# mic-rud/Learned-Compression-of-Point-Cloud-Geometry-and-Attributes

Measured on AMD Instinct MI355X. Metric: encode+decode Mpoints/sec, higher is better.
Workload: dtype f32

## Files before the change

### include/pcc_hip.h

```cpp
#ifndef PCC_HIP_H
#define PCC_HIP_H

#include <stdint.h>

#ifdef __cplusplus
extern "C" {
#endif

#define PCC_OK 0
#define PCC_ERR_ARG (-1)
#define PCC_ERR_HIP (-2)
#define PCC_ERR_UNSUPPORTED (-3)
#define PCC_ERR_DATA (-4)

#define PCC_ACT_NONE 0
#define PCC_ACT_RELU 1
#define PCC_ACT_LEAKY_RELU 2

int pcc_version(void);
const char* pcc_last_error(void);
int pcc_device_count(void);
int pcc_device_name(int dev, char* out, int out_len);

int64_t pcc_hash_capacity(int64_t n);
// ... 17 lines not shown
int pcc_children(const int32_t* coords, int64_t n, int32_t ts, int32_t ksize, uint64_t* keys,
                 int32_t* vals, int64_t cap, int32_t* scratch, int32_t* out_coords,
                 int64_t* out_count, void* stream);

int pcc_augment_rotate(const int32_t* coords, int64_t n, const float* rot, int32_t nbatch, float half,
                       uint64_t* keys, int32_t* vals, int64_t cap, int32_t* scratch, int32_t* out_coords,
                       int32_t* out_src, int64_t* out_count, void* stream);

int32_t pcc_color_jitter_chunk(void);
int64_t pcc_color_jitter_scratch_bytes(int64_t n, int32_t nbatch);
int pcc_color_jitter(const float* rgb, int64_t n, const int64_t* offsets, int32_t nbatch, const float* params,
                     const int32_t* order, float* out, void* scratch, int64_t scratch_bytes, void* stream);

int pcc_voxelize(const float* xyz, const int32_t* batch, int64_t n, int32_t nbatch, const float* attr, int32_t c,
                 float origin_x, float origin_y, float origin_z, float voxel, int32_t rounding, uint64_t* keys,
                 int32_t* vals, int64_t cap, int32_t* scratch, int32_t* out_coords, int32_t* out_first,
                 int32_t* out_npts, int64_t* out_sum, int32_t* out_row, int64_t* out_count, void* stream);

int pcc_kernel_map(const int32_t* out_coords, int64_t n_out, const uint64_t* in_keys,
                   const int32_t* in_vals, int64_t in_cap, int32_t ksize, int32_t step,
                   int32_t sign, int32_t* nbr, uint32_t* row_mask, int64_t* pair_count,
                   void* stream);

int pcc_pair_count(const uint32_t* row_mask, int64_t n_out, int64_t* pair_count, void* stream);

int64_t pcc_order_scratch_bytes(int64_t n);
int pcc_order_rows_by_mask(const uint32_t* row_mask, const int32_t* coords, int64_t n,
                           int32_t block_log2, int32_t tensor_stride, int32_t* order, uint32_t* group_mask32,
                           void* scratch, int64_t scratch_bytes, void* stream);
int pcc_permute_map_rows(const int32_t* nbr, const int32_t* order, int64_t n, int32_t K, int32_t* nbr_sorted, void* stream);

int64_t pcc_small_map_max(void);
int32_t pcc_small_paths(int32_t mask);
int pcc_small_kernel_map(const int32_t* out_coords, int64_t n_out, const uint64_t* in_keys, const int32_t* in_vals, int64_t in_cap,
                         int32_t ksize, int32_t step, int32_t sign, int32_t* nbr, uint32_t* row_mask, int32_t* order,
                         uint32_t* group_mask32, void* scratch, int64_t scratch_bytes, void* stream);

int64_t pcc_conv_packed_elems(int32_t K, int32_t cin, int32_t cout);
int pcc_conv_pack_weights(const float* w, int32_t K, int32_t cin, int32_t cout, float* w_packed,
                          void* stream);
int pcc_conv_fwd(const float* fin, int64_t n_in, int32_t cin, const float* w, const float* w_packed,
                 const float* bias, const int32_t* nbr, const int32_t* order,
                 const uint32_t* group_mask32, int32_t K, float* fout, int64_t n_out, int32_t cout,
                 int32_t act, const float* film, const float* residual, void* stream);

int64_t pcc_conv_small_max(int64_t workgroups);

int pcc_conv_kernel_name(int32_t mode, int64_t n_in, int32_t cin, int32_t cout, int64_t n_out, int32_t K, int32_t has_nbr,
                         char* buf, int32_t len);

int64_t pcc_conv_packed_elems_bf16(int32_t K, int32_t cin, int32_t cout);
int pcc_conv_pack_weights_bf16(const float* w, int32_t K, int32_t cin, int32_t cout, uint16_t* w_packed, void* stream);
// ... 13 lines not shown
int64_t pcc_conv_packed_elems_x3(int32_t K, int32_t cin, int32_t cout);
int pcc_conv_pack_weights_x3(const float* w, int32_t K, int32_t cin, int32_t cout, uint16_t* w_packed, void* stream);
int pcc_conv_fwd_x3(const float* fin, int64_t n_in, int32_t cin, const uint16_t* w_packed, const float* bias,
                    const int32_t* nbr, const int32_t* order, const uint32_t* group_mask32, int32_t K, float* fout,
                    int64_t n_out, int32_t cout, int32_t act, const float* film, const float* residual, void* stream);

int pcc_im2col_thin(const float* fin, int32_t cin, const int32_t* nbr, int64_t n_out, int32_t K, float* out, int32_t k2,
                    void* stream);

int pcc_gather_sum_fwd(const float* scores, int32_t ld, const int32_t* nbr, int32_t K, int32_t cout,
                       const float* bias, float* out, int64_t n_out, int32_t act, void* stream);

int pcc_gather_rows(const float* src, int32_t c, const int32_t* idx, int64_t n, float* out,
                    int32_t accumulate, void* stream);

int pcc_scatter_rows(const float* src, int32_t c, const int32_t* idx, int64_t n, float* out,
                     void* stream);
int pcc_scatter_add_rows(const float* src, int32_t c, const int32_t* idx, int64_t n, float* out,
                         void* stream);

int pcc_compact_rows(const uint8_t* mask, int64_t n, const int32_t* coords, int32_t* out_coords,
                     const float* feats, int32_t c, float* out_feats, int32_t* new_index,
                     int32_t* scratch, int64_t* out_count, void* stream);

int64_t pcc_topk_state_elems(int32_t nbatch);
int pcc_topk_mask(const float* logits, int32_t ld, const int32_t* coords, int64_t n, int32_t nbatch,
                  const int32_t* k, uint8_t* mask, int32_t* state, void* stream);

int pcc_count_per_batch(const int32_t* coords, int64_t n, int32_t nbatch, int32_t* counts, void* stream);

int64_t pcc_sort_scratch_bytes(int64_t n);
int pcc_sort_coords(const int32_t* coords, int64_t n, int32_t* perm, void* scratch,
                    int64_t scratch_bytes, void* stream);

int pcc_kernel_map_transpose(const int32_t* nbr, int64_t n_out, int32_t K, int64_t n_in, int32_t* nbr_t,
                             uint32_t* row_mask_t, void* stream);
int64_t pcc_conv_wgrad_scratch_elems(int32_t K, int32_t cin, int32_t cout);
int pcc_conv_wgrad(const float* fin, int64_t n_in, int32_t cin, const float* dy, int64_t n_out, int32_t cout,
                   const int32_t* nbr, const int32_t* order, const uint32_t* group_mask32, int32_t K, float* dw,
                   float* scratch, int64_t scratch_elems, void* stream);
int pcc_conv_wgrad_kernel_name(int32_t bf16, int32_t K, int32_t cin, int32_t cout, int64_t n_out, char* buf, int32_t len,
                               int32_t* split, int32_t* partials);
int pcc_conv_wgrad_bf16(const uint16_t* fin, int64_t n_in, int32_t cin, const uint16_t* dy, int64_t n_out, int32_t cout,
                        const int32_t* nbr, const int32_t* order, const uint32_t* group_mask32, int32_t K, float* dw,
                        float* scratch, int64_t scratch_elems, void* stream);

// ... 116 lines not shown
```

### learned-compression-of-point-cloud-geometry-and-attributes_amd/blocks.py

```python
import os

import torch
import torch.nn as nn

from . import _threads
from . import sparse as sp
from .sparse import (ACT_NONE, ACT_RELU, ConvChain, CoordMap, MinkowskiConvolution,
                     MinkowskiGenerativeConvolutionTranspose, MinkowskiPruning, MinkowskiReLU, SparseTensor)


class _NonNegativeParametrizer(nn.Module):
    def __init__(self, minimum=0.0, reparam_offset=2 ** -18):
        super().__init__()
        pedestal = float(reparam_offset) ** 2
        self.register_buffer("pedestal", torch.tensor([pedestal]))
        self.lower_bound = _Bound((float(minimum) + pedestal) ** 0.5)


class _Bound(nn.Module):
    def __init__(self, bound):
        super().__init__()
        self.register_buffer("bound", torch.tensor([float(bound)]))


# ... 24 lines not shown

    def forward(self, x, condition):
        if condition.map is x.map:
            film = condition.F
        else:
            film = condition.features_at_coordinates(x.C)
        N = x.F.shape[1]
        if film.shape[1] == 2 and N != 1:
            film = torch.cat([film[:, :1].expand(-1, N), film[:, 1:].expand(-1, N)], dim=1).contiguous()
        h = self.conv_1(x, last_film=film if self.scale else None)
        return self.conv_2(h, last_residual=x.F)


def _start_prefetch(x_map, done_key, job, handoffs):
    if os.environ.get("PCC_PREFETCH_MAPS", "1") == "0" or torch.is_grad_enabled() or x_map._cache.get(done_key):
        return False
    dev = x_map.device
    main = torch.cuda.current_stream(dev)
    st = _threads.current()
    skey = (dev, main.cuda_stream)
    side = st.side_streams.get(skey)
    if side is None:
        side = st.side_streams[skey] = torch.cuda.Stream(device=dev)
    x_map.table()
    side.wait_stream(main)

    def run():
        try:
            with torch.cuda.stream(side):
                job(side)
        except BaseException as e:
            for h in handoffs:
                h.fail(e)
            raise

    if x_map.n >= PREFETCH_THREAD_MIN_ROWS:
        x_map._cache[("prefetch_job",)] = st.job_thread("pcc-map-prefetch", dev).submit(run)
    else:
        run()
    x_map._cache[done_key] = True
    return True


PREFETCH_THREAD_MIN_ROWS = 8192


def prefetch_up_maps(x_map):
    first = _threads.Handoff()

    def job(side):
        cand = x_map.up(3)
        x_map.mfma_kernel_map(cand, 3, True)
        first.set(side.record_event())
        cand.mfma_kernel_map(cand, 3)
        cand.kernel_map(cand, 3)
# ... 37 lines not shown
    last = level == -1 or level >= len(syncs)
    try:
        ev = (syncs[-1] if last else syncs[level - 1]).wait()
    except BaseException:
        x_map._cache.pop(("analysis_syncs",), None)
        x_map._cache.pop(("prefetch_job",), None)
        raise
    torch.cuda.current_stream(x_map.device).wait_event(ev)
    if last:
        x_map._cache.pop(("analysis_syncs",), None)
        _join_prefetch(x_map)


def _join_prefetch_first(x_map):
    first = x_map._cache.pop(("prefetch_first",), None)
    if first is None:
        return
    try:
        ev = first.wait()
    except BaseException:
        x_map._cache.pop(("prefetch_job",), None)
        raise
    torch.cuda.current_stream(x_map.device).wait_event(ev)


def _join_prefetch(x_map):
    x_map._cache.pop(("prefetch_first",), None)
    done = x_map._cache.pop(("prefetch_job",), None)
    if done is not None:
        done.wait()
    ev = x_map._cache.pop(("prefetch_event",), None)
    if ev is not None:
        torch.cuda.current_stream(x_map.device).wait_event(ev)


class GenerativeUpBlock(nn.Module):

    def __init__(self, N_in, N_out, predict=False, dense=True, condition_ablation=None):
        super().__init__()
        self.dense = dense
        self.condition_ablation = condition_ablation
        self.conv = MinkowskiGenerativeConvolutionTranspose(in_channels=N_in, out_channels=N_out, kernel_size=3,
                                                            stride=2, bias=True, dimension=3)
        self.conv_2 = ConvChain(_conv(N_out, N_out), MinkowskiReLU(), _conv(N_out, N_out))
        self.prune = MinkowskiPruning()
        self.predict = predict
        if predict:
            self.occ_predict = ConvChain(_conv(N_out, N_out), MinkowskiReLU(), _conv(N_out, N_out))

    def forward(self, x, coords=None, k=None, full_predictions=False):
        if not self.predict:
            return self._follow(x, coords)
        in_map = x.map
        _join_prefetch_first(in_map)
        x = self.conv(x)
        _join_prefetch(in_map)
        if self.dense and self.condition_ablation is None:
            x = self.conv_2(x)
        pred = self.occ_predict(x, last_out_channels=None if full_predictions else 1)
        nb = x.map._nbatch if x.map._nbatch is not None else x.map.nbatch
        mask = sp.topk_mask(pred.F, pred.C, k, nb)
        kept = min(max(int(k[0]), 0), x.map.n) if nb == 1 and len(k) == 1 and not torch.is_grad_enabled() else None
        coords_kept, feats_kept, _, _ = sp.compact_rows(mask, x.C, x.F, expected=kept)
        up_map = CoordMap(coords_kept, x.map.stride, nbatch=x.map._nbatch)
        x = SparseTensor(feats_kept, coordinate_map=up_map)
        if not self.dense and self.condition_ablation is None:
            x = self.conv_2(x)
        return x, pred, up_map

    def _follow(self, Q, up_map):
        if not isinstance(up_map, CoordMap):
            up_map = CoordMap(sp._as_int_coords(up_map), Q.map.stride // 2, nbatch=Q.map._nbatch)
        return self.conv(Q, out_map=up_map)


class ConditionEncoder(nn.Module):

    def __init__(self, C_in, N_scales, N_features, condition_ablation=None):
        super().__init__()
        self.num_stages = len(N_scales)
        self.condition_ablation = condition_ablation
        self.pre_conv = ConvChain(_conv(C_in, N_features[0]), MinkowskiReLU())
        self.conv_layers = nn.ModuleList()
        self.predict_layers = nn.ModuleList()
        self.down_layers = nn.ModuleList()
        for i in range(self.num_stages):
            down = _conv(N_features[i], N_features[i + 1], 3, 2)
# ... 34 lines not shown
```

### learned-compression-of-point-cloud-geometry-and-attributes_amd/csrc/coords.hip

```cpp
#include <stdarg.h>
#include <stdio.h>
#include <stdlib.h>

#include "common.h"
#include "first_rows.h"
#include "sort.h"

namespace pcc {

static thread_local char g_err[512] = "";
void set_error(const char* fmt, ...) {
    va_list ap;
    va_start(ap, fmt);
    vsnprintf(g_err, sizeof(g_err), fmt, ap);
    va_end(ap);
}
const char* last_error() { return g_err; }

constexpr int SCAN_BLOCK = 256;
constexpr int SCAN_ITEMS = 4;
constexpr int SCAN_TILE = SCAN_BLOCK * SCAN_ITEMS;

__device__ __forceinline__ int wave_inclusive_scan(int v, int lane) {
#pragma unroll
    for (int d = 1; d < 64; d <<= 1) {
        const int t = __shfl_up(v, d, 64);
        if (lane >= d) v += t;
    }
// ... 396 lines not shown
            kk[i] = keys[sl];
            vv[i] = vals[sl];
        }
        int idx = -1;
        bool open = true;
        const int lane_slots = (int)((mask + TABLE_PROBE_STEP) / TABLE_PROBE_STEP);
#pragma unroll
        for (int i = 0; i < 4; ++i) {
            if (!open) break;
            if (i + 1 >= lane_slots) break;
            if (kk[i] == key) { idx = vv[i]; open = false; }
            else if (kk[i] == KEY_EMPTY) { idx = -1; open = false; }
        }
        if (open) idx = table_find(keys, vals, mask, shift, key);
        nbr[row0 * 27 + e] = idx;
        if (idx >= 0) { atomicOr(&rm[lr], 1u << k); ++myhits; }
    }
    if (myhits) atomicAdd(&hits_s, myhits);
    __syncthreads();
    if (row_mask && threadIdx.x < nrows) row_mask[row0 + threadIdx.x] = rm[threadIdx.x];
    if (threadIdx.x == 0 && pair_count && !row_mask && hits_s) atomicAdd(pair_count, (unsigned long long)hits_s);
}

__global__ __launch_bounds__(256) void pair_count_kernel(const uint32_t* __restrict__ row_mask, int64_t n,
                                                         unsigned long long* __restrict__ pair_count) {
    __shared__ unsigned long long ws[4];
    unsigned long long v = 0;
    for (int64_t i = (int64_t)blockIdx.x * 256 + threadIdx.x; i < n; i += (int64_t)gridDim.x * 256) v += __popc(row_mask[i]);
#pragma unroll
    for (int d = 32; d >= 1; d >>= 1) v += __shfl_xor(v, d, 64);
    if ((threadIdx.x & 63) == 0) ws[threadIdx.x >> 6] = v;
    __syncthreads();
    if (threadIdx.x == 0) {
        const unsigned long long t = ws[0] + ws[1] + ws[2] + ws[3];
        if (t) atomicAdd(pair_count, t);
    }
}

__global__ __launch_bounds__(256) void gather_rows_kernel(const float* __restrict__ src, int c,
                                                          const int32_t* __restrict__ idx, int64_t n,
                                                          float* __restrict__ out, int accumulate) {
    const int64_t total = n * c;
    for (int64_t e = (int64_t)blockIdx.x * blockDim.x + threadIdx.x; e < total; e += (int64_t)gridDim.x * blockDim.x) {
        const int64_t r = e / c;
        const int col = (int)(e - r * c);
        const int32_t s = idx[r];
// ... 16 lines not shown

__global__ __launch_bounds__(256) void scatter_add_rows_kernel(const float* __restrict__ src, int c,
                                                               const int32_t* __restrict__ idx, int64_t n,
                                                               float* __restrict__ out) {
    const int64_t total = n * c;
    for (int64_t e = (int64_t)blockIdx.x * blockDim.x + threadIdx.x; e < total; e += (int64_t)gridDim.x * blockDim.x) {
        const int64_t r = e / c;
        const int col = (int)(e - r * c);
        const int32_t d = idx[r];
        if (d >= 0) atomicAdd(&out[(int64_t)d * c + col], src[e]);
    }
}

__global__ __launch_bounds__(256) void mask_to_flags(const uint8_t* __restrict__ mask, int64_t n,
                                                     int32_t* __restrict__ flags) {
    const int64_t i = (int64_t)blockIdx.x * blockDim.x + threadIdx.x;
    if (i < n) flags[i] = mask[i] ? 1 : 0;
}

__global__ __launch_bounds__(256) void compact_index_kernel(const uint8_t* __restrict__ mask,
                                                            const int32_t* __restrict__ pos, int64_t n,
                                                            const int32_t* __restrict__ coords,
                                                            int32_t* __restrict__ out_coords,
                                                            int32_t* __restrict__ new_index) {
    const int64_t i = (int64_t)blockIdx.x * blockDim.x + threadIdx.x;
    if (i >= n) return;
    const bool keep = mask[i] != 0;
    const int32_t p = pos[i];
    if (new_index) new_index[i] = keep ? p : -1;
    if (keep && coords) reinterpret_cast<int4*>(out_coords)[p] = reinterpret_cast<const int4*>(coords)[i];
}

__global__ __launch_bounds__(256) void compact_feats_kernel(const uint8_t* __restrict__ mask,
                                                            const int32_t* __restrict__ pos, int64_t n, int c,
                                                            const float* __restrict__ feats,
                                                            float* __restrict__ out_feats, int vec) {
    if (vec) {
        const int c4 = c >> 2;
        const int64_t total = n * c4;
        const float4* src = reinterpret_cast<const float4*>(feats);
        float4* dst = reinterpret_cast<float4*>(out_feats);
        for (int64_t e = (int64_t)blockIdx.x * blockDim.x + threadIdx.x; e < total; e += (int64_t)gridDim.x * blockDim.x) {
            const int64_t r = e / c4;
            if (mask[r]) dst[(int64_t)pos[r] * c4 + (e - r * c4)] = src[e];
        }
        return;
    }
    const int64_t total = n * c;
    for (int64_t e = (int64_t)blockIdx.x * blockDim.x + threadIdx.x; e < total; e += (int64_t)gridDim.x * blockDim.x) {
        const int64_t r = e / c;
        if (mask[r]) out_feats[(int64_t)pos[r] * c + (e - r * c)] = feats[e];
    }
// ... 111 lines not shown
    const int in_stride = sign > 0 ? step : 2 * step;
    const int pitch = sign > 0 ? 0 : 2 * step;
    const bool pow2 = pitch == 0 || (pitch & (pitch - 1)) == 0;
    unsigned long long* pc = reinterpret_cast<unsigned long long*>(pair_count);
    const uint64_t tmask = (uint64_t)(in_cap - 1);
    const int tshift = grid_shift_of(in_stride);
    const unsigned nb = blocks_for(n_out, 64);
    hipStream_t st = as_stream(stream);
    if (ksize == 3) {
        if (pow2) hipLaunchKernelGGL(kernel_map27_kernel<true>, dim3(nb), dim3(256), 0, st, out_coords, n_out, in_keys, in_vals, tmask, tshift,
                                     sign * step, pitch, nbr, row_mask, pc);
        else hipLaunchKernelGGL(kernel_map27_kernel<false>, dim3(nb), dim3(256), 0, st, out_coords, n_out, in_keys, in_vals, tmask, tshift,
                                sign * step, pitch, nbr, row_mask, pc);
    } else {
        hipLaunchKernelGGL(kernel_map_kernel, dim3(nb), dim3(256), 0, st, out_coords, n_out, in_keys, in_vals, tmask, tshift, ksize, K,
                           sign * step, pitch, nbr, row_mask, pc);
    }
    if (pair_count && row_mask)
        hipLaunchKernelGGL(pair_count_kernel, dim3(blocks_for(n_out, 256 * 16, 512)), dim3(256), 0, st, row_mask, n_out, pc);
    PCC_LAUNCH_CHECK();
    return PCC_OK;
}

int pcc_pair_count(const uint32_t* row_mask, int64_t n_out, int64_t* pair_count, void* stream) {
    PCC_REQUIRE(pair_count != nullptr, "pcc_pair_count: no output");
    hipStream_t st = as_stream(stream);
    PCC_CHECK_HIP(hipMemsetAsync(pair_count, 0, sizeof(int64_t), st));
    if (n_out <= 0) return PCC_OK;
    hipLaunchKernelGGL(pair_count_kernel, dim3(blocks_for(n_out, 256 * 16, 512)), dim3(256), 0, st, row_mask, n_out,
                       reinterpret_cast<unsigned long long*>(pair_count));
    PCC_LAUNCH_CHECK();
    return PCC_OK;
}

int pcc_gather_rows(const float* src, int32_t c, const int32_t* idx, int64_t n, float* out, int32_t accumulate,
                    void* stream) {
    if (n <= 0 || c <= 0) return PCC_OK;
    hipLaunchKernelGGL(gather_rows_kernel, dim3(blocks_for(n * c, 256, 65536)), dim3(256), 0, as_stream(stream), src, c,
                       idx, n, out, accumulate);
    PCC_LAUNCH_CHECK();
    return PCC_OK;
}

int pcc_scatter_rows(const float* src, int32_t c, const int32_t* idx, int64_t n, float* out, void* stream) {
    if (n <= 0 || c <= 0) return PCC_OK;
    hipLaunchKernelGGL(scatter_rows_kernel, dim3(blocks_for(n * c, 256, 65536)), dim3(256), 0, as_stream(stream), src,
                       c, idx, n, out);
    PCC_LAUNCH_CHECK();
    return PCC_OK;
}

int pcc_scatter_add_rows(const float* src, int32_t c, const int32_t* idx, int64_t n, float* out, void* stream) {
    if (n <= 0 || c <= 0) return PCC_OK;
    hipLaunchKernelGGL(scatter_add_rows_kernel, dim3(blocks_for(n * c, 256, 65536)), dim3(256), 0, as_stream(stream), src,
                       c, idx, n, out);
    PCC_LAUNCH_CHECK();
    return PCC_OK;
}

int pcc_compact_rows(const uint8_t* mask, int64_t n, const int32_t* coords, int32_t* out_coords, const float* feats,
                     int32_t c, float* out_feats, int32_t* new_index, int32_t* scratch, int64_t* out_count,
                     void* stream) {
    hipStream_t st = as_stream(stream);
    if (n <= 0) {
        PCC_CHECK_HIP(hipMemsetAsync(out_count, 0, sizeof(int64_t), st));
        return PCC_OK;
    }
    int32_t* flags = scratch;
    int32_t* block_sums = scratch + n;
    hipLaunchKernelGGL(mask_to_flags, dim3(blocks_for(n, 256)), dim3(256), 0, st, mask, n, flags);
    int rc = exclusive_scan(flags, n, flags, block_sums, out_count, st);
    if (rc) return rc;
    if (coords || new_index)
        hipLaunchKernelGGL(compact_index_kernel, dim3(blocks_for(n, 256)), dim3(256), 0, st, mask, flags, n, coords,
                           out_coords, new_index);
    if (feats && c > 0)
    {
        const int vec = (c & 3) == 0 && ((reinterpret_cast<uintptr_t>(feats) | reinterpret_cast<uintptr_t>(out_feats)) & 15) == 0;
        hipLaunchKernelGGL(compact_feats_kernel, dim3(blocks_for(vec ? n * (c / 4) : n * c, 256, 65536)), dim3(256), 0, st,
                           mask, flags, n, c, feats, out_feats, vec);
    }
    PCC_LAUNCH_CHECK();
    return PCC_OK;
}

int pcc_count_per_batch(const int32_t* coords, int64_t n, int32_t nbatch, int32_t* counts, void* stream) {
    hipStream_t st = as_stream(stream);
    PCC_REQUIRE(nbatch >= 1, "pcc_count_per_batch: nbatch must be >= 1");
    PCC_CHECK_HIP(hipMemsetAsync(counts, 0, sizeof(int32_t) * nbatch, st));
    if (n > 0) hipLaunchKernelGGL(count_batch_kernel, dim3(blocks_for(n, 256)), dim3(256), 0, st, coords, n, nbatch, counts);
    PCC_LAUNCH_CHECK();
    return PCC_OK;
}

}
```

### learned-compression-of-point-cloud-geometry-and-attributes_amd/csrc/select.hip

```cpp
#include <stdlib.h>

#include "common.h"
#include "sort_small.h"

namespace pcc {

constexpr int TK_STRIDE = 264;
constexpr int TK_LDS_BATCHES = 16;

__device__ __forceinline__ uint32_t float_key(float v) {
    if (v != v) return 0xFFFFFFFFu;
    if (v == 0.0f) v = 0.0f;
    const uint32_t u = __float_as_uint(v);
    return (u & 0x80000000u) ? ~u : (u | 0x80000000u);
}

struct Key96 { uint32_t w[3]; };

__device__ __forceinline__ Key96 make_key(float logit, int4 c) {
    const uint64_t lo = ~pack_key(c.x, c.y, c.z, c.w);
    Key96 k;
    k.w[0] = float_key(logit);
    k.w[1] = (uint32_t)(lo >> 32);
    k.w[2] = (uint32_t)lo;
    return k;
// ... 214 lines not shown
    const int t = threadIdx.x;
    if (t < 8) st[t] = 0;
    __syncthreads();
    if (t == 0) topk_state_init(st, k[0]);
    __syncthreads();
    topk_rounds(0, 12, n, st, h, &total_s, [&](int i, int pass, Key96& key) {
        const int4 c = pass < 4 ? make_int4(0, 0, 0, 0) : reinterpret_cast<const int4*>(coords)[i];
        if (c.x != 0) return false;
        key = make_key(logits[(int64_t)i * ld], c);
        return true;
    });
    const int nb = st[2];
    for (int i = t; i < n; i += 1024) {
        const int4 c = reinterpret_cast<const int4*>(coords)[i];
        uint8_t m = 0;
        if (c.x == 0 && nb <= 12) m = cmp_prefix(make_key(logits[(int64_t)i * ld], c), st, nb) >= 0 ? 1 : 0;
        mask[i] = m;
    }
    for (int i = t; i < TK_STRIDE; i += 1024) state[i] = i < 8 ? st[i] : 0;
}

__global__ __launch_bounds__(256) void mask_bit_counts_kernel(const uint32_t* __restrict__ row_mask, int64_t n,
                                                              uint32_t* __restrict__ counts) {
    __shared__ unsigned c[27];
    if (threadIdx.x < 27) c[threadIdx.x] = 0u;
    __syncthreads();
    unsigned mine[27];
#pragma unroll
    for (int b = 0; b < 27; ++b) mine[b] = 0u;
    for (int64_t i0 = (int64_t)blockIdx.x * 256; i0 < n; i0 += (int64_t)gridDim.x * 256) {
        const int64_t i = i0 + threadIdx.x;
        const uint32_t m = (i < n) ? row_mask[i] : 0u;
#pragma unroll
        for (int b = 0; b < 27; ++b) mine[b] += (unsigned)__popcll(__ballot((m >> b) & 1u));
    }
    if ((threadIdx.x & 63) == 0) {
#pragma unroll
        for (int b = 0; b < 27; ++b)
            if (mine[b]) atomicAdd(&c[b], mine[b]);
    }
    __syncthreads();
    if (threadIdx.x < 27 && c[threadIdx.x]) atomicAdd(&counts[threadIdx.x], c[threadIdx.x]);
}

__device__ __forceinline__ void order_bit_positions(const uint32_t* __restrict__ counts, int* pos_s) {
    if (threadIdx.x < 27) {
        const uint32_t mine = counts[threadIdx.x];
        int rank = 0;
        for (int b = 0; b < 27; ++b) {
            const uint32_t o = counts[b];
            rank += (o < mine || (o == mine && b < (int)threadIdx.x)) ? 1 : 0;
        }
        pos_s[threadIdx.x] = 26 - rank;
    }
    __syncthreads();
}

__device__ __forceinline__ uint32_t order_key_of(uint32_t m, const int* pos_s) {
    uint32_t key = 0u;
#pragma unroll
    for (int b = 0; b < 27; ++b) key |= ((m >> b) & 1u) << pos_s[b];
    return 0x7FFFFFFu - key;
}

__global__ __launch_bounds__(256) void order_keys32_kernel(const uint32_t* __restrict__ row_mask, int64_t n,
// ... 218 lines not shown
            }
            hipLaunchKernelGGL(topk_tail_kernel, dim3(1), dim3(1024), 0, st, logits, ld, coords, n, state);
            hipLaunchKernelGGL(topk_write_mask, dim3(blocks_for(n, 256)), dim3(256), 0, st, logits, ld, coords, n, nbatch,
                               state, mask);
            PCC_LAUNCH_CHECK();
            return PCC_OK;
        }
        for (int pass = 0; pass < 12; ++pass) {
            hipLaunchKernelGGL(topk_hist, dim3(nb), dim3(256), 0, st, logits, ld, coords, n, nbatch, pass, state);
            hipLaunchKernelGGL(topk_pick, dim3(nbatch), dim3(256), 0, st, pass, state);
        }
        hipLaunchKernelGGL(topk_write_mask, dim3(blocks_for(n, 256)), dim3(256), 0, st, logits, ld, coords, n, nbatch,
                           state, mask);
    }
    PCC_LAUNCH_CHECK();
    return PCC_OK;
}

int64_t pcc_order_scratch_bytes(int64_t n) { return pcc_sort_scratch_bytes(n); }

int pcc_order_rows_by_mask(const uint32_t* row_mask, const int32_t* coords, int64_t n, int32_t block_log2,
                           int32_t tensor_stride, int32_t* order, uint32_t* group_mask32, void* scratch, int64_t scratch_bytes,
                           void* stream) {
    if (n <= 0) return PCC_OK;
    PCC_REQUIRE(n < (1ll << 31), "pcc_order_rows_by_mask: too many rows");
    PCC_REQUIRE(block_log2 < 0 || coords != nullptr, "pcc_order_rows_by_mask: block ordering needs coordinates");
    PCC_REQUIRE(block_log2 <= 10, "pcc_order_rows_by_mask: block_log2 out of range");
    PCC_REQUIRE(tensor_stride >= 1, "pcc_order_rows_by_mask: bad tensor stride");
    PCC_REQUIRE(scratch_bytes >= pcc_sort_scratch_bytes(n), "pcc_order_rows_by_mask: scratch too small");
    hipStream_t st = as_stream(stream);
    const SortScratch s = carve_sort_scratch(scratch, n);
    if (small_path_enabled(0) && block_log2 < 0 && n <= RS_SMALL_N) {
        rs_small_dispatch(rs_small_rounds((int)n), [&](auto r) {
            hipLaunchKernelGGL(order_small_kernel<decltype(r)::value>, dim3(1), dim3(RS_SMALL_THREADS), 0, st, row_mask, (int)n,
                               static_cast<uint32_t*>(s.keys_a), static_cast<uint32_t*>(s.keys_b), s.vals_x, order);
        });
    } else {
        uint32_t* bit_counts = s.tail;
        PCC_CHECK_HIP(hipMemsetAsync(bit_counts, 0, 27 * sizeof(uint32_t), st));
        hipLaunchKernelGGL(mask_bit_counts_kernel, dim3(blocks_for(n, 256 * 16, 512)), dim3(256), 0, st, row_mask, n, bit_counts);
        const int begin = 0, end = block_log2 >= 0 ? 64 : 27;
        const int digit_bits = block_log2 >= 0 ? 8 : radix_sort_order_digit_bits(n);
        const bool in_b = radix_sort_result_in_b(begin, end, digit_bits);
        int32_t* va = in_b ? s.vals_x : order;
        int32_t* vb = in_b ? order : s.vals_x;
        int rc;
        if (block_log2 < 0) {
            uint32_t* ka = static_cast<uint32_t*>(s.keys_a);
            hipLaunchKernelGGL(order_keys32_kernel, dim3(blocks_for(n, 256)), dim3(256), 0, st, row_mask, n, bit_counts, ka);
            rc = radix_sort_pairs_u32(ka, static_cast<uint32_t*>(s.keys_b), va, vb, true, n, begin, end, s.counters, st, digit_bits);
        } else {
            uint64_t* ka = static_cast<uint64_t*>(s.keys_a);
            hipLaunchKernelGGL(order_keys64_kernel, dim3(blocks_for(n, 256)), dim3(256), 0, st, row_mask, coords, n, block_log2, tensor_stride,
                               bit_counts, ka);
            rc = radix_sort_pairs_u64(ka, static_cast<uint64_t*>(s.keys_b), va, vb, true, n, begin, end, s.counters, st);
        }
        if (rc) return rc;
    }
    hipLaunchKernelGGL(group_masks_kernel, dim3(blocks_for(n, 256)), dim3(256), 0, st, order, row_mask, n, group_mask32);
    PCC_LAUNCH_CHECK();
    return PCC_OK;
}

// ... 55 lines not shown
```

### learned-compression-of-point-cloud-geometry-and-attributes_amd/sparse.py

```python
import ctypes
import functools
import math
import weakref

import os

import torch
import torch.nn as nn

from . import _lib, _threads
from ._lib import PCC, check, ptr

ACT_NONE, ACT_RELU, ACT_LRELU = PCC.ACT_NONE, PCC.ACT_RELU, PCC.ACT_LEAKY_RELU


def _require_cuda(t):
    if not t.is_cuda:
        raise RuntimeError("libpcc_hip operators need tensors on an MI355X device (got a CPU tensor); "
                           "there is no CPU fallback")


COORD_PROFILER = None


# ... 91 lines not shown
        if self._val is None:
            out = torch.empty(1, dtype=torch.int64, device=self._mask.device)
            check(_lib.lib().pcc_pair_count(ptr(self._mask), self._mask.shape[0], ptr(out), _lib.stream()))
            self._val = int(out.item())
        return self._val

    __int__ = item

    def __float__(self):
        return float(self.item())


def _same_map(kept, out_map, self_map):
    if kept is None:
        return out_map is self_map
    return kept() is out_map


def _order_buffers(n, dev):
    return (torch.empty(n, dtype=torch.int32, device=dev), torch.empty((n + 31) // 32, dtype=torch.int32, device=dev),
            torch.empty(_lib.lib().pcc_order_scratch_bytes(n), dtype=torch.uint8, device=dev))


def _execution_order(row_mask, coords, n, stride):
    order, gmask, scratch = _order_buffers(n, coords.device)
    check(_lib.lib().pcc_order_rows_by_mask(ptr(row_mask), ptr(coords), n, ORDER_BLOCK_LOG2, stride, ptr(order), ptr(gmask),
                                            ptr(scratch), scratch.shape[0], _lib.stream()))
    return order, gmask


class CoordMap:

    def __init__(self, coords, stride=1, table=None, nbatch=None):
        _require_cuda(coords)
        assert coords.dtype == torch.int32 and coords.dim() == 2 and coords.shape[1] == 4
        self.coords = coords.contiguous()
        self.stride = int(stride)
        self._table = table
        self._nbatch = nbatch
        self._cache = {}
        self._dup_word = None

    @property
    def n(self):
        return self.coords.shape[0]

    @property
    def device(self):
        return self.coords.device

    @property
    def nbatch(self):
        if self._nbatch is None:
            self._nbatch = int(self.coords[:, 0].max().item()) + 1 if self.n else 1
        return self._nbatch

    def table(self):
        if self._table is None:
            L = _lib.lib()
            cap = L.pcc_hash_capacity(self.n)
            keys = torch.empty(cap, dtype=torch.int64, device=self.device)
            vals = torch.empty(cap, dtype=torch.int32, device=self.device)
            ev = _cp_begin()
            check(L.pcc_hash_build(ptr(self.coords), self.n, ptr(keys), ptr(vals), cap, self.stride, ptr(self._dup_word), _lib.stream()))
            _cp_end(ev, "hash_build", self.n, 28 * self.n + 12 * cap)
            self._table = (keys, vals, cap)
        return self._table

    def count_duplicates(self):
        assert self._table is None
        self._dup_word = torch.empty(1, dtype=torch.int32, device=self.device)

    def duplicates(self):
        return 0 if self._dup_word is None or self._table is None else int(self._dup_word.item())

    def lookup(self, query):
        keys, vals, cap = self.table()
        q = _as_int_coords(query)
        out = torch.empty(q.shape[0], dtype=torch.int32, device=self.device)
        ev = _cp_begin()
# ... 64 lines not shown
        nbr, row_mask, pairs = self.kernel_map(out_map, ksize, transposed)
        n_out = nbr.shape[0]
        ev = _cp_begin()
        order, gmask = _execution_order(row_mask, out_map.coords, n_out, out_map.stride)
        _cp_end(ev, "execution_order", n_out, 100 * n_out)
        return self._keep_for(out_map, key, nbr, order, gmask, pairs)

    def _small_ordered_kernel_map(self, out_map, ksize, transposed, key):
        L = _lib.lib()
        keys, vals, cap = self.table()
        n_out, K, dev = out_map.n, ksize ** 3, self.device
        nbr = torch.empty((n_out, K), dtype=torch.int32, device=dev)
        row_mask = torch.empty(n_out, dtype=torch.int32, device=dev)
        order, gmask, scratch = _order_buffers(n_out, dev)
        step = self.stride // 2 if transposed else self.stride
        ev = _cp_begin()
        check(L.pcc_small_kernel_map(ptr(out_map.coords), n_out, ptr(keys), ptr(vals), cap, ksize, step, -1 if transposed else 1,
                                     ptr(nbr), ptr(row_mask), ptr(order), ptr(gmask), ptr(scratch), scratch.shape[0], _lib.stream()))
        pairs = PairCount(row_mask)
        _cp_end(ev, "small_map+order", n_out, (120 + 12 * K) * n_out)
        self._keep_for(out_map, ("kmap", id(out_map), ksize, transposed), nbr, row_mask, pairs)
        return self._keep_for(out_map, key, nbr, order, gmask, pairs)

    def position_ordered_table(self, out_map, ksize, transposed=False):
        key = ("okmap_sorted", id(out_map), ksize, transposed, ORDER_BLOCK_LOG2)
        hit = self._cached_for(out_map, key)
        if hit is not None:
            return hit
        nbr, order, gmask, pairs = self.ordered_kernel_map(out_map, ksize, transposed)
        nbr_sorted = torch.empty_like(nbr)
        check(_lib.lib().pcc_permute_map_rows(ptr(nbr), ptr(order), nbr.shape[0], nbr.shape[1], ptr(nbr_sorted), _lib.stream()))
        return self._keep_for(out_map, key, nbr_sorted, order, gmask, pairs)

    def transposed_ordered_map(self, out_map, ksize, transposed=False):
        key = ("tmap", id(out_map), ksize, transposed, ORDER_BLOCK_LOG2)
        hit = self._cached_for(out_map, key)
        if hit is not None:
            return hit
        nbr, _, _ = self.kernel_map(out_map, ksize, transposed)
        n_out, K = nbr.shape
        nbr_t = torch.empty((self.n, K), dtype=torch.int32, device=self.device)
        mask_t = torch.empty(self.n, dtype=torch.int32, device=self.device)
        check(_lib.lib().pcc_kernel_map_transpose(ptr(nbr), n_out, K, self.n, ptr(nbr_t), ptr(mask_t), _lib.stream()))
        return self._keep_for(out_map, key, nbr_t, *_execution_order(mask_t, self.coords, self.n, self.stride))

    def conv_map(self, out_map, ksize, transposed, cin, adjoint=False):
# ... 147 lines not shown
        ctx.save_for_backward(new_index)
        if out_c is None:
            out_c = new_index.new_empty((0, 4))
        ctx.mark_non_differentiable(out_c, new_index)
        return out_f, out_c, new_index

    @staticmethod
    def backward(ctx, g, _gc, _gi):
        (new_index,) = ctx.saved_tensors
        g = g.contiguous()
        d = torch.empty((new_index.shape[0], g.shape[1]), dtype=torch.float32, device=g.device)
        check(_lib.lib().pcc_gather_rows(ptr(g), g.shape[1], ptr(new_index), new_index.shape[0], ptr(d), 0, _lib.stream()))
        return d, None, None


def scatter_rows(src, idx, n_out):
    if _tracked(src):
        return _ScatterRowsFn.apply(src, idx.contiguous(), n_out)
    out = torch.zeros((n_out, src.shape[1]), dtype=torch.float32, device=src.device)
    check(_lib.lib().pcc_scatter_rows(ptr(src), src.shape[1], ptr(idx), idx.shape[0], ptr(out), _lib.stream()))
    return out


def compact_rows(mask, coords=None, feats=None, want_index=False, expected=None):
    if _tracked(feats):
        feats_k, coords_k, new_index = _CompactFeatsFn.apply(feats, mask, coords)
        return (coords_k if coords is not None else None), feats_k, (new_index if want_index else None), feats_k.shape[0]
    L = _lib.lib()
    n = mask.shape[0]
    dev = mask.device
    scratch = torch.empty(L.pcc_scan_scratch_elems(n), dtype=torch.int32, device=dev)
    known = expected is not None and n > 0 and not CHECK_EXPECTED_COUNTS
    count, word = (None, None) if known else _host_count()
    out_c = torch.empty((n, 4), dtype=torch.int32, device=dev) if coords is not None else None
    c = feats.shape[1] if feats is not None else 0
    out_f = torch.empty((n, c), dtype=torch.float32, device=dev) if feats is not None else None
    new_index = torch.empty(n, dtype=torch.int32, device=dev) if want_index else None
    ev = _cp_begin()
    check(L.pcc_compact_rows(ptr(mask), n, ptr(coords), ptr(out_c), ptr(feats), c, ptr(out_f), ptr(new_index),
                             ptr(scratch), ptr(count), _lib.stream()))
    if known:
        m = int(expected)
    else:
        m = _read_count(word, dev)
        if expected is not None and m != int(expected):
            raise RuntimeError(f"compact_rows: {m} rows kept where the caller expected {int(expected)}")
    _cp_end(ev, "prune", n, 13 * n + (2 * (16 if coords is not None else 0) + 8 * c) * m)
    return (out_c[:m] if out_c is not None else None, out_f[:m] if out_f is not None else None, new_index, m)


def topk_mask(logits, coords, k_per_batch, nbatch):
    L = _lib.lib()
    n = logits.shape[0]
    dev = logits.device
    ks = [int(v) for v in k_per_batch]
    assert len(ks) == nbatch, (len(ks), nbatch)
    if nbatch == 1:
        k = torch.full((1,), ks[0], dtype=torch.int32, device=dev)
    else:
        k = torch.tensor(ks, dtype=torch.int32).pin_memory().to(dev, non_blocking=True)
    state = torch.empty(L.pcc_topk_state_elems(nbatch), dtype=torch.int32, device=dev)
    mask = torch.empty(n, dtype=torch.uint8, device=dev)
    ev = _cp_begin()
    check(L.pcc_topk_mask(ptr(logits), logits.stride(0), ptr(coords), n, nbatch, ptr(k), ptr(mask), ptr(state),
                          _lib.stream()))
    _cp_end(ev, "top_k", n, 37 * n)
    return mask


def conv_forward(x_feats, in_map, out_map, layer, ksize, transposed=False, act=ACT_NONE, film=None,
                 residual=None, out_channels=None):
# ... 389 lines not shown
```

### learned-compression-of-point-cloud-geometry-and-attributes_amd/transforms.py

```python
import torch
import torch.nn as nn

from . import sparse as sp
from .blocks import join_analysis_level, prefetch_analysis_maps, prefetch_up_maps, ConditionEncoder, GenerativeUpBlock, ScaledBlock, _conv
from .sparse import ConvChain, CoordMap, MinkowskiConvolution, MinkowskiReLU, SparseTensor


def _align(Q, target_map):
    if Q.map is target_map:
        return Q
    if Q.map.n != target_map.n or Q.map.stride != target_map.stride:
        return None
    idx = target_map.lookup(Q.C)
    if not bool((idx >= 0).all()):
        return None
    return SparseTensor(sp.scatter_rows(Q.F, idx, target_map.n), coordinate_map=target_map)


class AnalysisTransform(nn.Module):

    def __init__(self, config):
        super().__init__()
        C_in, N1, N2, N3 = config["C_in"], config["N1"], config["N2"], config["N3"]
        self.condition_ablation = config.get("condition_ablation")
# ... 88 lines not shown
        aligned = _align(Q, x.map)
        if aligned is not None:
            Q = aligned
        if self.cond_conv:
            Q_plus = self.cond_conv(x)
            if Q.map is x.map:
                Q = SparseTensor(Q.F + Q_plus.F, coordinate_map=Q.map)
            else:
                feats = sp.gather_rows(Q_plus.F, Q_plus.map.lookup(Q.C), out=Q.F.clone(), accumulate=True)
                Q = SparseTensor(feats, coordinate_map=Q.map)

        x = self.pre_conv(x)
        Q = self.q_pre_conv(Q)

        predictions = []
        ups = (self.up_1, self.up_2, self.up_3)
        q_ups = (self.q_up_1, self.q_up_2, self.q_up_3)
        q_predicts = (self.q_predict_1, self.q_predict_2, self.q_predict_3)
        scales = (self.scale_1, self.scale_2, self.scale_3)
        for i in range(3):
            prefetch_up_maps(x.map)
            beta_gamma = q_predicts[i](Q, last_out_map=x.map)
            x = scales[i](x, beta_gamma)
            x, pred, up_map = ups[i](x, k=k[i], full_predictions=full_pred)
            Q = q_ups[i](Q, up_map)
            predictions.append(pred)

        x = self.post_conv(x)

        if coords is not None:
            points_1 = coords.map.down()
            points_2 = points_1.down()
            points = [SparseTensor(coordinate_map=points_2), SparseTensor(coordinate_map=points_1), coords]
            return x, points, predictions
        return x
```

Measured before the change: 9.050.

## Derive pruned kernel maps from superset maps instead of rebuilding via hashing

After top-k pruning in the generative up blocks, the kernel maps for the pruned coordinate set are now built by gathering rows from the already-built superset neighbor map and remapping indices. The offset counts are computed in the same kernel and passed to the execution-order sort, so it skips its separate counting pass. The hash table build for adopted maps moves onto the prefetch side stream. On the last stage in inference the unused Q upsample is skipped. This removes repeated hash lookups per pruned level, at the cost of extra index buffers and more complex cross-stream handoffs.

```diff
diff --git a/include/pcc_hip.h b/include/pcc_hip.h
--- a/include/pcc_hip.h
+++ b/include/pcc_hip.h
@@ -63,12 +63,19 @@
                    int32_t sign, int32_t* nbr, uint32_t* row_mask, int64_t* pair_count,
                    void* stream);
 
+int pcc_kernel_map_from_superset(const int32_t* nbr_sup, int64_t n_sup, const int32_t* old_index,
+                                 const int32_t* new_index, int64_t n_sub, int32_t K, int32_t remap, int32_t* nbr_sub,
+                                 uint32_t* row_mask, uint32_t* offset_counts, void* stream);
+
 int pcc_pair_count(const uint32_t* row_mask, int64_t n_out, int64_t* pair_count, void* stream);
 
 int64_t pcc_order_scratch_bytes(int64_t n);
 int pcc_order_rows_by_mask(const uint32_t* row_mask, const int32_t* coords, int64_t n,
                            int32_t block_log2, int32_t tensor_stride, int32_t* order, uint32_t* group_mask32,
                            void* scratch, int64_t scratch_bytes, void* stream);
+int pcc_order_rows_by_mask_counts(const uint32_t* row_mask, const int32_t* coords, int64_t n,
+                                  int32_t block_log2, int32_t tensor_stride, int32_t* order, uint32_t* group_mask32,
+                                  void* scratch, int64_t scratch_bytes, const uint32_t* offset_counts, void* stream);
 int pcc_permute_map_rows(const int32_t* nbr, const int32_t* order, int64_t n, int32_t K, int32_t* nbr_sorted, void* stream);
 
 int64_t pcc_small_map_max(void);
@@ -128,6 +135,9 @@
 int pcc_compact_rows(const uint8_t* mask, int64_t n, const int32_t* coords, int32_t* out_coords,
                      const float* feats, int32_t c, float* out_feats, int32_t* new_index,
                      int32_t* scratch, int64_t* out_count, void* stream);
+int pcc_compact_rows_index(const uint8_t* mask, int64_t n, const int32_t* coords, int32_t* out_coords,
+                           const float* feats, int32_t c, float* out_feats, int32_t* new_index, int32_t* old_index,
+                           int32_t* scratch, int64_t* out_count, void* stream);
 
 int64_t pcc_topk_state_elems(int32_t nbatch);
 int pcc_topk_mask(const float* logits, int32_t ld, const int32_t* coords, int64_t n, int32_t nbatch,
diff --git a/learned-compression-of-point-cloud-geometry-and-attributes_amd/blocks.py b/learned-compression-of-point-cloud-geometry-and-attributes_amd/blocks.py
--- a/learned-compression-of-point-cloud-geometry-and-attributes_amd/blocks.py
+++ b/learned-compression-of-point-cloud-geometry-and-attributes_amd/blocks.py
@@ -70,15 +70,22 @@
     side = st.side_streams.get(skey)
     if side is None:
         side = st.side_streams[skey] = torch.cuda.Stream(device=dev)
-    x_map.table()
+    table_built = None
+    if x_map._table is None and x_map._cache.get(("adopted",)):
+        table_built = x_map._cache[("table_handoff",)] = _threads.Handoff()
+    else:
+        x_map.table()
     side.wait_stream(main)
 
     def run():
         try:
             with torch.cuda.stream(side):
+                if table_built is not None:
+                    x_map._build_table()
+                    table_built.set(side.record_event())
                 job(side)
         except BaseException as e:
-            for h in handoffs:
+            for h in handoffs + ([] if table_built is None else [table_built]):
                 h.fail(e)
             raise
 
@@ -162,6 +169,7 @@
         x_map._cache.pop(("prefetch_job",), None)
         raise
     torch.cuda.current_stream(x_map.device).wait_event(ev)
+    x_map._cache.pop(("table_handoff",), None)
 
 
 def _join_prefetch(x_map):
@@ -172,6 +180,7 @@
     ev = x_map._cache.pop(("prefetch_event",), None)
     if ev is not None:
         torch.cuda.current_stream(x_map.device).wait_event(ev)
+        x_map._cache.pop(("table_handoff",), None)
 
 
 class GenerativeUpBlock(nn.Module):
@@ -188,7 +197,7 @@
         if predict:
             self.occ_predict = ConvChain(_conv(N_out, N_out), MinkowskiReLU(), _conv(N_out, N_out))
 
-    def forward(self, x, coords=None, k=None, full_predictions=False):
+    def forward(self, x, coords=None, k=None, full_predictions=False, q_follows=True):
         if not self.predict:
             return self._follow(x, coords)
         in_map = x.map
@@ -201,8 +210,12 @@
         nb = x.map._nbatch if x.map._nbatch is not None else x.map.nbatch
         mask = sp.topk_mask(pred.F, pred.C, k, nb)
         kept = min(max(int(k[0]), 0), x.map.n) if nb == 1 and len(k) == 1 and not torch.is_grad_enabled() else None
-        coords_kept, feats_kept, _, _ = sp.compact_rows(mask, x.C, x.F, expected=kept)
+        derive = sp.pruned_maps_enabled() and not torch.is_grad_enabled()
+        coords_kept, feats_kept, new_index, _, *old_index = sp.compact_rows(mask, x.C, x.F, want_index=derive, expected=kept,
+                                                                            want_old_index=derive)
         up_map = CoordMap(coords_kept, x.map.stride, nbatch=x.map._nbatch)
+        if derive:
+            up_map.adopt_maps_from(x.map, in_map if q_follows else None, old_index[0], new_index, 3)
         x = SparseTensor(feats_kept, coordinate_map=up_map)
         if not self.dense and self.condition_ablation is None:
             x = self.conv_2(x)
diff --git a/learned-compression-of-point-cloud-geometry-and-attributes_amd/csrc/coords.hip b/learned-compression-of-point-cloud-geometry-and-attributes_amd/csrc/coords.hip
--- a/learned-compression-of-point-cloud-geometry-and-attributes_amd/csrc/coords.hip
+++ b/learned-compression-of-point-cloud-geometry-and-attributes_amd/csrc/coords.hip
@@ -4,6 +4,7 @@
 
 #include "common.h"
 #include "first_rows.h"
+#include "offset_counts.h"
 #include "sort.h"
 
 namespace pcc {
@@ -446,6 +447,71 @@
     if (threadIdx.x == 0 && pair_count && !row_mask && hits_s) atomicAdd(pair_count, (unsigned long long)hits_s);
 }
 
+constexpr unsigned MAP_SUBSET_GROUPS = 2048;
+template <int KT>
+__global__ __launch_bounds__(256) void map_from_superset_kernel(const int32_t* __restrict__ nbr_sup, int64_t n_sup,
+                                                                const int32_t* __restrict__ old_index,
+                                                                const int32_t* __restrict__ new_index, int64_t n_sub, int k_rt,
+                                                                int remap, int32_t* __restrict__ nbr_sub,
+                                                                uint32_t* __restrict__ row_mask, uint32_t* __restrict__ counts) {
+    const int K = KT ? KT : k_rt;
+    __shared__ int32_t src_row[64];
+    __shared__ unsigned rm[64];
+    __shared__ unsigned c27[OFFSET_COUNTS];
+    if (threadIdx.x < OFFSET_COUNTS) c27[threadIdx.x] = 0u;
+    unsigned mine[OFFSET_COUNTS];
+    offset_counts_clear(mine);
+    const int64_t tiles = (n_sub + 63) / 64;
+    constexpr int U = 7;
+    for (int64_t tile = blockIdx.x; tile < tiles; tile += gridDim.x) {
+        const int64_t row0 = tile * 64;
+        const int nrows = (int)((n_sub - row0 < 64) ? (n_sub - row0) : 64);
+        if (threadIdx.x < 64) {
+            int32_t s = -1;
+            if ((int)threadIdx.x < nrows) {
+                s = old_index[row0 + threadIdx.x];
+                if ((uint64_t)(int64_t)s >= (uint64_t)n_sup) s = -1;
+            }
+            src_row[threadIdx.x] = s;
+            rm[threadIdx.x] = 0u;
+        }
+        __syncthreads();
+        const int total = nrows * K;
+        for (int e0 = threadIdx.x; e0 < total; e0 += 256 * U) {
+            int32_t v[U];
+#pragma unroll
+            for (int j = 0; j < U; ++j) {
+                const int e = e0 + 256 * j;
+                v[j] = -1;
+                if (e < total) {
+                    const int lr = e / K;
+                    const int32_t s = src_row[lr];
+                    if (s >= 0) v[j] = nbr_sup[(int64_t)s * K + (e - lr * K)];
+                }
+            }
+            if (remap) {
+#pragma unroll
+                for (int j = 0; j < U; ++j) v[j] = (v[j] >= 0 && (int64_t)v[j] < n_sup) ? new_index[v[j]] : -1;
+            }
+#pragma unroll
+            for (int j = 0; j < U; ++j) {
+                const int e = e0 + 256 * j;
+                if (e >= total) continue;
+                nbr_sub[row0 * K + e] = v[j];
+                if (v[j] >= 0) { const int lr = e / K; atomicOr(&rm[lr], 1u << (e - lr * K)); }
+            }
+        }
+        __syncthreads();
+        if (threadIdx.x < 64) {
+            const uint32_t m = rm[threadIdx.x];
+            if ((int)threadIdx.x < nrows) row_mask[row0 + threadIdx.x] = m;
+            if (counts) offset_counts_add(mine, m);
+        }
+    }
+    __syncthreads();
+    if (counts) offset_counts_flush(mine, c27, counts);
+}
+
 __global__ __launch_bounds__(256) void pair_count_kernel(const uint32_t* __restrict__ row_mask, int64_t n,
                                                          unsigned long long* __restrict__ pair_count) {
     __shared__ unsigned long long ws[4];
@@ -508,12 +574,14 @@
                                                             const int32_t* __restrict__ pos, int64_t n,
                                                             const int32_t* __restrict__ coords,
                                                             int32_t* __restrict__ out_coords,
-                                                            int32_t* __restrict__ new_index) {
+                                                            int32_t* __restrict__ new_index,
+                                                            int32_t* __restrict__ old_index) {
     const int64_t i = (int64_t)blockIdx.x * blockDim.x + threadIdx.x;
     if (i >= n) return;
     const bool keep = mask[i] != 0;
     const int32_t p = pos[i];
     if (new_index) new_index[i] = keep ? p : -1;
+    if (keep && old_index) old_index[p] = (int32_t)i;
     if (keep && coords) reinterpret_cast<int4*>(out_coords)[p] = reinterpret_cast<const int4*>(coords)[i];
 }
 
@@ -671,6 +739,26 @@
     return PCC_OK;
 }
 
+int pcc_kernel_map_from_superset(const int32_t* nbr_sup, int64_t n_sup, const int32_t* old_index, const int32_t* new_index,
+                                 int64_t n_sub, int32_t K, int32_t remap, int32_t* nbr_sub, uint32_t* row_mask,
+                                 uint32_t* offset_counts, void* stream) {
+    PCC_REQUIRE(K >= 1 && K <= 27, "pcc_kernel_map_from_superset: K %d out of range 1..27", K);
+    PCC_REQUIRE(n_sub >= 0 && n_sub <= n_sup, "pcc_kernel_map_from_superset: %lld subset rows of %lld", (long long)n_sub, (long long)n_sup);
+    PCC_REQUIRE(n_sup < (1ll << 31), "pcc_kernel_map_from_superset: too many rows (%lld)", (long long)n_sup);
+    PCC_REQUIRE(nbr_sup != nullptr && old_index != nullptr && nbr_sub != nullptr && row_mask != nullptr,
+                "pcc_kernel_map_from_superset: null argument");
+    PCC_REQUIRE(!remap || new_index != nullptr, "pcc_kernel_map_from_superset: remap needs new_index");
+    if (n_sub == 0) return PCC_OK;
+    const unsigned nb = blocks_for(n_sub, 64, MAP_SUBSET_GROUPS);
+    hipStream_t st = as_stream(stream);
+    if (K == 27) hipLaunchKernelGGL(map_from_superset_kernel<27>, dim3(nb), dim3(256), 0, st, nbr_sup, n_sup, old_index, new_index, n_sub,
+                                    K, remap, nbr_sub, row_mask, offset_counts);
+    else hipLaunchKernelGGL(map_from_superset_kernel<0>, dim3(nb), dim3(256), 0, st, nbr_sup, n_sup, old_index, new_index, n_sub, K,
+                            remap, nbr_sub, row_mask, offset_counts);
+    PCC_LAUNCH_CHECK();
+    return PCC_OK;
+}
+
 int pcc_pair_count(const uint32_t* row_mask, int64_t n_out, int64_t* pair_count, void* stream) {
     PCC_REQUIRE(pair_count != nullptr, "pcc_pair_count: no output");
     hipStream_t st = as_stream(stream);
@@ -710,6 +798,12 @@
 int pcc_compact_rows(const uint8_t* mask, int64_t n, const int32_t* coords, int32_t* out_coords, const float* feats,
                      int32_t c, float* out_feats, int32_t* new_index, int32_t* scratch, int64_t* out_count,
                      void* stream) {
+    return pcc_compact_rows_index(mask, n, coords, out_coords, feats, c, out_feats, new_index, nullptr, scratch, out_count, stream);
+}
+
+int pcc_compact_rows_index(const uint8_t* mask, int64_t n, const int32_t* coords, int32_t* out_coords, const float* feats,
+                           int32_t c, float* out_feats, int32_t* new_index, int32_t* old_index, int32_t* scratch,
+                           int64_t* out_count, void* stream) {
     hipStream_t st = as_stream(stream);
     if (n <= 0) {
         PCC_CHECK_HIP(hipMemsetAsync(out_count, 0, sizeof(int64_t), st));
@@ -720,9 +814,9 @@
     hipLaunchKernelGGL(mask_to_flags, dim3(blocks_for(n, 256)), dim3(256), 0, st, mask, n, flags);
     int rc = exclusive_scan(flags, n, flags, block_sums, out_count, st);
     if (rc) return rc;
-    if (coords || new_index)
+    if (coords || new_index || old_index)
         hipLaunchKernelGGL(compact_index_kernel, dim3(blocks_for(n, 256)), dim3(256), 0, st, mask, flags, n, coords,
-                           out_coords, new_index);
+                           out_coords, new_index, old_index);
     if (feats && c > 0)
     {
         const int vec = (c & 3) == 0 && ((reinterpret_cast<uintptr_t>(feats) | reinterpret_cast<uintptr_t>(out_feats)) & 15) == 0;
diff --git a/learned-compression-of-point-cloud-geometry-and-attributes_amd/csrc/offset_counts.h b/learned-compression-of-point-cloud-geometry-and-attributes_amd/csrc/offset_counts.h
--- /dev/null
+++ b/learned-compression-of-point-cloud-geometry-and-attributes_amd/csrc/offset_counts.h
@@ -0,0 +1,28 @@
+#pragma once
+#include "common.h"
+
+namespace pcc {
+
+constexpr int OFFSET_COUNTS = 27;
+
+__device__ __forceinline__ void offset_counts_clear(unsigned (&mine)[OFFSET_COUNTS]) {
+#pragma unroll
+    for (int b = 0; b < OFFSET_COUNTS; ++b) mine[b] = 0u;
+}
+
+__device__ __forceinline__ void offset_counts_add(unsigned (&mine)[OFFSET_COUNTS], uint32_t m) {
+#pragma unroll
+    for (int b = 0; b < OFFSET_COUNTS; ++b) mine[b] += (unsigned)__popcll(__ballot((m >> b) & 1u));
+}
+
+__device__ __forceinline__ void offset_counts_flush(const unsigned (&mine)[OFFSET_COUNTS], unsigned* c, uint32_t* __restrict__ counts) {
+    if ((threadIdx.x & 63) == 0) {
+#pragma unroll
+        for (int b = 0; b < OFFSET_COUNTS; ++b)
+            if (mine[b]) atomicAdd(&c[b], mine[b]);
+    }
+    __syncthreads();
+    if (threadIdx.x < OFFSET_COUNTS && c[threadIdx.x]) atomicAdd(&counts[threadIdx.x], c[threadIdx.x]);
+}
+
+}
diff --git a/learned-compression-of-point-cloud-geometry-and-attributes_amd/csrc/select.hip b/learned-compression-of-point-cloud-geometry-and-attributes_amd/csrc/select.hip
--- a/learned-compression-of-point-cloud-geometry-and-attributes_amd/csrc/select.hip
+++ b/learned-compression-of-point-cloud-geometry-and-attributes_amd/csrc/select.hip
@@ -1,6 +1,7 @@
 #include <stdlib.h>
 
 #include "common.h"
+#include "offset_counts.h"
 #include "sort_small.h"
 
 namespace pcc {
@@ -261,25 +262,16 @@
 
 __global__ __launch_bounds__(256) void mask_bit_counts_kernel(const uint32_t* __restrict__ row_mask, int64_t n,
                                                               uint32_t* __restrict__ counts) {
-    __shared__ unsigned c[27];
-    if (threadIdx.x < 27) c[threadIdx.x] = 0u;
-    __syncthreads();
-    unsigned mine[27];
-#pragma unroll
-    for (int b = 0; b < 27; ++b) mine[b] = 0u;
+    __shared__ unsigned c[OFFSET_COUNTS];
+    if (threadIdx.x < OFFSET_COUNTS) c[threadIdx.x] = 0u;
+    __syncthreads();
+    unsigned mine[OFFSET_COUNTS];
+    offset_counts_clear(mine);
     for (int64_t i0 = (int64_t)blockIdx.x * 256; i0 < n; i0 += (int64_t)gridDim.x * 256) {
         const int64_t i = i0 + threadIdx.x;
-        const uint32_t m = (i < n) ? row_mask[i] : 0u;
-#pragma unroll
-        for (int b = 0; b < 27; ++b) mine[b] += (unsigned)__popcll(__ballot((m >> b) & 1u));
-    }
-    if ((threadIdx.x & 63) == 0) {
-#pragma unroll
-        for (int b = 0; b < 27; ++b)
-            if (mine[b]) atomicAdd(&c[b], mine[b]);
-    }
-    __syncthreads();
-    if (threadIdx.x < 27 && c[threadIdx.x]) atomicAdd(&counts[threadIdx.x], c[threadIdx.x]);
+        offset_counts_add(mine, (i < n) ? row_mask[i] : 0u);
+    }
+    offset_counts_flush(mine, c, counts);
 }
 
 __device__ __forceinline__ void order_bit_positions(const uint32_t* __restrict__ counts, int* pos_s) {
@@ -544,6 +536,13 @@
 int pcc_order_rows_by_mask(const uint32_t* row_mask, const int32_t* coords, int64_t n, int32_t block_log2,
                            int32_t tensor_stride, int32_t* order, uint32_t* group_mask32, void* scratch, int64_t scratch_bytes,
                            void* stream) {
+    return pcc_order_rows_by_mask_counts(row_mask, coords, n, block_log2, tensor_stride, order, group_mask32, scratch, scratch_bytes,
+                                         nullptr, stream);
+}
+
+int pcc_order_rows_by_mask_counts(const uint32_t* row_mask, const int32_t* coords, int64_t n, int32_t block_log2,
+                                  int32_t tensor_stride, int32_t* order, uint32_t* group_mask32, void* scratch,
+                                  int64_t scratch_bytes, const uint32_t* offset_counts, void* stream) {
     if (n <= 0) return PCC_OK;
     PCC_REQUIRE(n < (1ll << 31), "pcc_order_rows_by_mask: too many rows");
     PCC_REQUIRE(block_log2 < 0 || coords != nullptr, "pcc_order_rows_by_mask: block ordering needs coordinates");
@@ -558,9 +557,12 @@
                                static_cast<uint32_t*>(s.keys_a), static_cast<uint32_t*>(s.keys_b), s.vals_x, order);
         });
     } else {
-        uint32_t* bit_counts = s.tail;
-        PCC_CHECK_HIP(hipMemsetAsync(bit_counts, 0, 27 * sizeof(uint32_t), st));
-        hipLaunchKernelGGL(mask_bit_counts_kernel, dim3(blocks_for(n, 256 * 16, 512)), dim3(256), 0, st, row_mask, n, bit_counts);
+        const uint32_t* bit_counts = offset_counts;
+        if (!bit_counts) {
+            PCC_CHECK_HIP(hipMemsetAsync(s.tail, 0, OFFSET_COUNTS * sizeof(uint32_t), st));
+            hipLaunchKernelGGL(mask_bit_counts_kernel, dim3(blocks_for(n, 256 * 16, 512)), dim3(256), 0, st, row_mask, n, s.tail);
+            bit_counts = s.tail;
+        }
         const int begin = 0, end = block_log2 >= 0 ? 64 : 27;
         const int digit_bits = block_log2 >= 0 ? 8 : radix_sort_order_digit_bits(n);
         const bool in_b = radix_sort_result_in_b(begin, end, digit_bits);
diff --git a/learned-compression-of-point-cloud-geometry-and-attributes_amd/sparse.py b/learned-compression-of-point-cloud-geometry-and-attributes_amd/sparse.py
--- a/learned-compression-of-point-cloud-geometry-and-attributes_amd/sparse.py
+++ b/learned-compression-of-point-cloud-geometry-and-attributes_amd/sparse.py
@@ -137,11 +137,15 @@
             torch.empty(_lib.lib().pcc_order_scratch_bytes(n), dtype=torch.uint8, device=dev))
 
 
-def _execution_order(row_mask, coords, n, stride):
+def _execution_order(row_mask, coords, n, stride, offset_counts=None):
     order, gmask, scratch = _order_buffers(n, coords.device)
-    check(_lib.lib().pcc_order_rows_by_mask(ptr(row_mask), ptr(coords), n, ORDER_BLOCK_LOG2, stride, ptr(order), ptr(gmask),
-                                            ptr(scratch), scratch.shape[0], _lib.stream()))
+    check(_lib.lib().pcc_order_rows_by_mask_counts(ptr(row_mask), ptr(coords), n, ORDER_BLOCK_LOG2, stride, ptr(order), ptr(gmask),
+                                                   ptr(scratch), scratch.shape[0], ptr(offset_counts), _lib.stream()))
     return order, gmask
+
+
+def pruned_maps_enabled():
+    return os.environ.get("PCC_PRUNED_MAPS", "1") != "0"
 
 
 class CoordMap:
@@ -171,6 +175,14 @@
         return self._nbatch
 
     def table(self):
+        pending = self._cache.get(("table_handoff",))
+        if pending is not None:
+            torch.cuda.current_stream(self.device).wait_event(pending.wait())
+        elif self._table is None:
+            self._build_table()
+        return self._table
+
+    def _build_table(self):
         if self._table is None:
             L = _lib.lib()
             cap = L.pcc_hash_capacity(self.n)
@@ -281,6 +293,42 @@
         self._keep_for(out_map, ("kmap", id(out_map), ksize, transposed), nbr, row_mask, pairs)
         return self._keep_for(out_map, key, nbr, order, gmask, pairs)
 
+    def adopt_maps_from(self, superset_map, parent_map, old_index, new_index, ksize=3, parent_order=False):
+        if not pruned_maps_enabled() or torch.is_grad_enabled():
+            return False
+        if 0 < self.n <= _small_map_max() and ksize in (2, 3) and ORDER_BLOCK_LOG2 < 0:
+            return False
+        K = ksize ** 3
+        sup = superset_map._cached_for(superset_map, ("kmap", id(superset_map), ksize, False))
+        if sup is None or sup[0].shape != (superset_map.n, K):
+            return False
+        self._derive_map(self, self, sup[0], old_index, new_index, ksize, False, True)
+        par = None if parent_map is None else parent_map._cached_for(superset_map, ("kmap", id(superset_map), ksize, True))
+        if par is not None and par[0].shape == (superset_map.n, K):
+            self._derive_map(parent_map, self, par[0], old_index, None, ksize, True, parent_order)
+        self._cache[("adopted",)] = True
+        return True
+
+    @staticmethod
+    def _derive_map(in_map, out_map, nbr_sup, old_index, new_index, ksize, transposed, ordered):
+        n, K, dev = out_map.n, ksize ** 3, out_map.device
+        nbr = torch.empty((n, K), dtype=torch.int32, device=dev)
+        row_mask = torch.empty(n, dtype=torch.int32, device=dev)
+        counts = torch.zeros(27, dtype=torch.int32, device=dev) if ordered and n else None
+        ev = _cp_begin()
+        if n:
+            check(_lib.lib().pcc_kernel_map_from_superset(ptr(nbr_sup), nbr_sup.shape[0], ptr(old_index), ptr(new_index), n, K,
+                                                          0 if new_index is None else 1, ptr(nbr), ptr(row_mask), ptr(counts),
+                                                          _lib.stream()))
+        pairs = PairCount(row_mask)
+        _cp_end(ev, "kernel_map_derived", n, lambda: 8 * n + 8 * K * n + (0 if new_index is None else 4 * int(pairs)))
+        in_map._keep_for(out_map, ("kmap", id(out_map), ksize, transposed), nbr, row_mask, pairs)
+        if ordered:
+            ev = _cp_begin()
+            order, gmask = _execution_order(row_mask, out_map.coords, n, out_map.stride, counts)
+            _cp_end(ev, "execution_order", n, 96 * n)
+            in_map._keep_for(out_map, ("okmap", id(out_map), ksize, transposed, ORDER_BLOCK_LOG2), nbr, order, gmask, pairs)
+
     def position_ordered_table(self, out_map, ksize, transposed=False):
         key = ("okmap_sorted", id(out_map), ksize, transposed, ORDER_BLOCK_LOG2)
         hit = self._cached_for(out_map, key)
@@ -474,8 +522,9 @@
     return out
 
 
-def compact_rows(mask, coords=None, feats=None, want_index=False, expected=None):
+def compact_rows(mask, coords=None, feats=None, want_index=False, expected=None, want_old_index=False):
     if _tracked(feats):
+        assert not want_old_index
         feats_k, coords_k, new_index = _CompactFeatsFn.apply(feats, mask, coords)
         return (coords_k if coords is not None else None), feats_k, (new_index if want_index else None), feats_k.shape[0]
     L = _lib.lib()
@@ -488,9 +537,10 @@
     c = feats.shape[1] if feats is not None else 0
     out_f = torch.empty((n, c), dtype=torch.float32, device=dev) if feats is not None else None
     new_index = torch.empty(n, dtype=torch.int32, device=dev) if want_index else None
+    old_index = torch.empty(n, dtype=torch.int32, device=dev) if want_old_index else None
     ev = _cp_begin()
-    check(L.pcc_compact_rows(ptr(mask), n, ptr(coords), ptr(out_c), ptr(feats), c, ptr(out_f), ptr(new_index),
-                             ptr(scratch), ptr(count), _lib.stream()))
+    check(L.pcc_compact_rows_index(ptr(mask), n, ptr(coords), ptr(out_c), ptr(feats), c, ptr(out_f), ptr(new_index), ptr(old_index),
+                                   ptr(scratch), ptr(count), _lib.stream()))
     if known:
         m = int(expected)
     else:
@@ -498,7 +548,8 @@
         if expected is not None and m != int(expected):
             raise RuntimeError(f"compact_rows: {m} rows kept where the caller expected {int(expected)}")
     _cp_end(ev, "prune", n, 13 * n + (2 * (16 if coords is not None else 0) + 8 * c) * m)
-    return (out_c[:m] if out_c is not None else None, out_f[:m] if out_f is not None else None, new_index, m)
+    res = (out_c[:m] if out_c is not None else None, out_f[:m] if out_f is not None else None, new_index, m)
+    return res + (old_index[:m],) if want_old_index else res
 
 
 def topk_mask(logits, coords, k_per_batch, nbatch):
diff --git a/learned-compression-of-point-cloud-geometry-and-attributes_amd/transforms.py b/learned-compression-of-point-cloud-geometry-and-attributes_amd/transforms.py
--- a/learned-compression-of-point-cloud-geometry-and-attributes_amd/transforms.py
+++ b/learned-compression-of-point-cloud-geometry-and-attributes_amd/transforms.py
@@ -134,8 +134,10 @@
             prefetch_up_maps(x.map)
             beta_gamma = q_predicts[i](Q, last_out_map=x.map)
             x = scales[i](x, beta_gamma)
-            x, pred, up_map = ups[i](x, k=k[i], full_predictions=full_pred)
-            Q = q_ups[i](Q, up_map)
+            q_follows = i + 1 < len(ups) or torch.is_grad_enabled()
+            x, pred, up_map = ups[i](x, k=k[i], full_predictions=full_pred, q_follows=q_follows)
+            if q_follows:
+                Q = q_ups[i](Q, up_map)
             predictions.append(pred)
 
         x = self.post_conv(x)
```

Result: no change. 9.061, median of 2 (+0.1%).
